# fverdoja/Fast-3D-Pointcloud-Segmentation

Hardware: AMD Instinct MI355X
Metric: Mpoints/sec segmented end-to-end, 1M-pt RGB-D frames (higher is better)
Workload: dtype f32

## Files before the change

### fast-3d-pointcloud-segmentation_amd/csrc/f3ds_algo.h

```cpp
#ifndef F3DS_ALGO_H_
#define F3DS_ALGO_H_

#include "f3ds_numerics.h"

namespace f3ds {

#define F3DS_MAX_SEED_EVENTS 48
struct SeedEvent {
    int trigger;
    int depth;
    double min[3];
    unsigned off[3];
};
struct SeedGrid {
    int n_events;
    int error;
    int defined;
    int depth;
    double res;
    double min[3], max[3];
    unsigned off[3];
    SeedEvent ev[F3DS_MAX_SEED_EVENTS];
};
F3DS_HD void a_seed_init(SeedGrid& g, float seed_res) {
// ... 126 lines not shown
    for (;;) {
        const int w = node[sp];
        const uint32_t h = s.owner[w];
        const float dw = s.dist[w];
        bool pushed = false, stolen = false;
        uint32_t g_cached = 0; bool cached_less = false;
        const bool ghosts_w = ghosts && memo[w] != (unsigned char)(T | F3DS_R_OPEN);
        for (int k = slot[sp]; k < 27; ++k) {
            int u = a_nbr_w(s, w, k);
            if (u < 0) continue;
            if (ghosts_w) {
                for (uint32_t gg = s.ghost_head[u]; gg != 0u; gg = s.ghost_next[gg])
                    if (gg < h && a_helper_dist(s, gg, w) < dw) { stolen = true; break; }
                if (stolen) break;
            }
            uint32_t g = s.owner[u];
            if (g == 0u || g >= h) continue;
            if (g != g_cached) { g_cached = g; cached_less = a_helper_dist(s, g, w) < dw; }
            if (!cached_less) continue;
            const unsigned char mu = memo[u];
            if (mu == (T | F3DS_R_TRUE)) { stolen = true; break; }
            if (mu == (T | F3DS_R_FALSE)) continue;
            slot[sp] = k + 1;
            if (sp + 1 >= F3DS_R_STACK) { *overflow = 1; return true; }
            ++sp; node[sp] = u; slot[sp] = 0;
            pushed = true;
            break;
        }
        if (pushed) continue;
        bool r = !stolen;
        for (;;) {
            memo[node[sp]] = (unsigned char)(T | (r ? F3DS_R_TRUE : F3DS_R_FALSE));
            if (sp == 0) return r;
            --sp;
            if (r) { r = false; continue; }
            break;
        }
    }
}
F3DS_HD bool a_eval_R(const SweepView& s, int w, unsigned char* memo, unsigned char tag, int* overflow, bool ghost_near = true) {
    const unsigned char T = (unsigned char)(tag << 2);
    {
        const unsigned char m0 = memo[w];
        if ((m0 & 0xFC) == T && (m0 & 3) != F3DS_R_OPEN) return (m0 & 3) == F3DS_R_TRUE;
        if (m0 == (unsigned char)(T | F3DS_R_OPEN)) ghost_near = false;
    }
    if (ghost_near && *s.n_ghosts != 0u) return a_eval_R_chain(s, w, memo, tag, overflow);
    const uint32_t h = s.owner[w];
    const float dw = s.dist[w];
    int nu[27]; uint32_t og[27];
    for (int k = 0; k < 27; ++k) nu[k] = a_nbr_w(s, w, k);
    for (int k = 0; k < 27; ++k) {
        const uint32_t g = s.owner[nu[k] >= 0 ? nu[k] : w];
        og[k] = (nu[k] >= 0 && g != 0u && g < h) ? g : 0u;
    }
    bool stolen = false, unknown = false;
    uint32_t last = 0;
    for (;;) {
        uint32_t g = 0xFFFFFFFFu;
        for (int k = 0; k < 27; ++k) if (og[k] > last && og[k] < g) g = og[k];
        if (g == 0xFFFFFFFFu) break;
        last = g;
        if (!(a_helper_dist(s, g, w) < dw)) continue;
        for (int k = 0; k < 27; ++k)
            if (og[k] == g) {
                const unsigned char mu = memo[nu[k]];
                if (mu == (T | F3DS_R_TRUE)) stolen = true;
                else if (mu != (T | F3DS_R_FALSE)) unknown = true;
            }
        if (stolen) break;
    }
    if (!stolen && unknown) return a_eval_R_chain(s, w, memo, tag, overflow);
    memo[w] = (unsigned char)(T | (stolen ? F3DS_R_FALSE : F3DS_R_TRUE));
    return !stolen;
}
#define F3DS_NO_NEXT 0x40000000u
F3DS_HD uint32_t a_umin(uint32_t a, uint32_t b) { return a < b ? a : b; }
F3DS_HD uint32_t a_umax(uint32_t a, uint32_t b) { return a > b ? a : b; }
F3DS_HD uint32_t a_next_label(const uint32_t x[27], uint32_t bias) {
    uint32_t m[9];
    for (int k = 0; k < 9; ++k) m[k] = a_umin(a_umin(x[3 * k] - bias, x[3 * k + 1] - bias), x[3 * k + 2] - bias);
    return a_umin(a_umin(a_umin(m[0], m[1]), m[2]), a_umin(a_umin(a_umin(m[3], m[4]), m[5]), a_umin(a_umin(m[6], m[7]), m[8])));
}
F3DS_HD bool a_has_thief_words(const SweepView& s, int w, uint32_t h, const uint32_t x[27]) {
    uint32_t y = a_next_label(x, 1u);
    uint32_t g = y + 1u;
    if (y >= F3DS_NO_NEXT || g >= h) return false;
    const float dw = s.dist[w];
    float wrow[12];
    a_load_row(s.vf + (size_t)w * 12, wrow);
    for (;;) {
        if (a_helper_dist_row(s, g, wrow) < dw) return true;
        const uint32_t last = g;
        y = a_next_label(x, last + 1u);
        g = y + last + 1u;
        if (y >= F3DS_NO_NEXT || g >= h) return false;
    }
}
F3DS_HD uint32_t a_thief_mask_words(const SweepView& s, int w, uint32_t h, const uint32_t x[27]) {
    uint32_t y = a_next_label(x, 1u);
    uint32_t g = y + 1u;
    if (y >= F3DS_NO_NEXT || g >= h) return 0u;
    const float dw = s.dist[w];
    float wrow[12];
    a_load_row(s.vf + (size_t)w * 12, wrow);
    uint32_t mask = 0u;
    for (;;) {
        if (a_helper_dist_row(s, g, wrow) < dw)
            for (int k = 0; k < 27; ++k) mask |= (x[k] == g ? 1u : 0u) << k;
        const uint32_t last = g;
        y = a_next_label(x, last + 1u);
        g = y + last + 1u;
        if (y >= F3DS_NO_NEXT || g >= h) return mask;
    }
}
F3DS_HD uint32_t a_thief_mask(const SweepView& s, int w) {
    const uint32_t h = s.owner[w];
    int nu[27]; uint32_t x[27];
    for (int k = 0; k < 27; ++k) nu[k] = a_nbr(s, w, k);
    for (int k = 0; k < 27; ++k) {
        const uint32_t g = s.owner[nu[k] >= 0 ? nu[k] : w];
        x[k] = nu[k] >= 0 ? g : 0u;
    }
    return a_thief_mask_words(s, w, h, x);
}
F3DS_HD bool a_ghost_steals(const SweepView& s, int w, uint32_t h) {
    const float dw = s.dist[w];
    for (int k = 0; k < 27; ++k) {
        const int u = a_nbr(s, w, k);
        if (u < 0) continue;
        for (uint32_t gg = s.ghost_head[u]; gg != 0u; gg = s.ghost_next[gg])
            if (gg < h && a_helper_dist(s, gg, w) < dw) return true;
    }
    return false;
}
#define F3DS_TMASK_GHOST 0x80000000u
F3DS_HD bool a_eval_R_mask(const SweepView& s, int w0, unsigned char* memo, unsigned char tag, const uint32_t* tmask, int* overflow) {
    const unsigned char T = (unsigned char)(tag << 2);
    {
        const unsigned char m0 = memo[w0];
        if ((m0 & 0xFC) == T && (m0 & 3) != F3DS_R_OPEN) return (m0 & 3) == F3DS_R_TRUE;
    }
    uint32_t mask0 = tmask[w0];
    if (mask0 & F3DS_TMASK_GHOST) {
        if (a_ghost_steals(s, w0, s.owner[w0])) { memo[w0] = (unsigned char)(T | F3DS_R_FALSE); return false; }
        mask0 &= ~F3DS_TMASK_GHOST;
    }
    bool stolen = false, unknown = false;
    for (uint32_t m = mask0; m != 0u; m &= m - 1u) {
        const int u = a_nbr_w(s, w0, (int)__builtin_ctz(m));
        const unsigned char mu = memo[u];
        if (mu == (unsigned char)(T | F3DS_R_TRUE)) stolen = true;
        else if (mu != (unsigned char)(T | F3DS_R_FALSE)) unknown = true;
    }
    if (stolen || !unknown) { memo[w0] = (unsigned char)(T | (stolen ? F3DS_R_FALSE : F3DS_R_TRUE)); return !stolen; }
    int node[F3DS_R_STACK];
    uint32_t rem[F3DS_R_STACK];
    int sp = 0;
    node[0] = w0; rem[0] = mask0;
    for (;;) {
        const int w = node[sp];
        bool pushed = false, st = false;
        while (rem[sp] != 0u) {
            const int k = (int)__builtin_ctz(rem[sp]);
            const int u = a_nbr_w(s, w, k);
            const unsigned char mu = memo[u];
            if (mu == (unsigned char)(T | F3DS_R_TRUE)) { st = true; break; }
            rem[sp] &= rem[sp] - 1u;
            if (mu == (unsigned char)(T | F3DS_R_FALSE)) continue;
            if (sp + 1 >= F3DS_R_STACK) { *overflow = 1; return true; }
            uint32_t mu_ = tmask[u];
            if (mu_ & F3DS_TMASK_GHOST) {
                if (a_ghost_steals(s, u, s.owner[u])) { memo[u] = (unsigned char)(T | F3DS_R_FALSE); continue; }
                mu_ &= ~F3DS_TMASK_GHOST;
            }
            ++sp; node[sp] = u; rem[sp] = mu_;
            pushed = true;
            break;
        }
        if (pushed) continue;
        bool r = !st;
        for (;;) {
            memo[node[sp]] = (unsigned char)(T | (r ? F3DS_R_TRUE : F3DS_R_FALSE));
            if (sp == 0) return r;
            --sp;
            if (r) { r = false; continue; }
            break;
        }
    }
}
F3DS_HD bool a_eval_R_step(const SweepView& s, const uint32_t* ownR, int w) {
    const uint32_t h = s.owner[w];
    if (h == 0u) return false;
    int nu[27]; uint32_t x[27];
    for (int k = 0; k < 27; ++k) nu[k] = a_nbr(s, w, k);
    for (int k = 0; k < 27; ++k) {
        const int u = nu[k] >= 0 ? nu[k] : w;
        const uint32_t g = s.owner[u], r = ownR[u];
        x[k] = (nu[k] >= 0 && (r & F3DS_OWNR_RTRUE)) ? g : 0u;
    }
    return !a_has_thief_words(s, w, h, x);
}
F3DS_HD bool a_has_thief(const SweepView& s, int w) {
    const uint32_t h = s.owner[w];
    int nu[27]; uint32_t x[27];
    for (int k = 0; k < 27; ++k) nu[k] = a_nbr(s, w, k);
    for (int k = 0; k < 27; ++k) {
        const uint32_t g = s.owner[nu[k] >= 0 ? nu[k] : w];
        x[k] = nu[k] >= 0 ? g : 0u;
    }
    return a_has_thief_words(s, w, h, x);
}
F3DS_HD void a_claim_words(const SweepView& s, int v, const uint32_t x[27], uint32_t* owner_out, float* dist_out) {
    uint32_t o = s.owner[v];
    float d = s.dist[v];
#if defined(F3DS_EXP_CLAIM_NOSEL)
    { uint32_t z = 0; for (int k = 0; k < 27; ++k) z |= x[k]; *owner_out = z == 0x7FFFFFFFu ? 1u : o; *dist_out = d; return; }
#endif
    float vrow[12];
    a_load_row(s.vf + (size_t)v * 12, vrow);
    uint32_t last = 0;
    for (;;) {
        const uint32_t y = a_next_label(x, F3DS_OWNR_RTRUE + last + 1u);
        if (y >= F3DS_NO_NEXT) break;
        const uint32_t g = y + last + 1u;
        last = g;
        if (g == o) continue;
#if defined(F3DS_EXP_CLAIM_NODIST)
        float dg = (float)g + vrow[0];
#else
        float dg = a_helper_dist_row(s, g, vrow);
#endif
        if (dg < d) { d = dg; o = g; }
    }
    *owner_out = o; *dist_out = d;
}
F3DS_HD void a_claim(const SweepView& s, const uint32_t* ownR, int v, uint32_t* owner_out, float* dist_out, unsigned char* ghost_done) {
    const bool ghosts = *s.n_ghosts != 0u;
    int nu[27]; uint32_t cand[27];
    for (int k = 0; k < 27; ++k) nu[k] = a_nbr(s, v, k);
    for (int k = 0; k < 27; ++k) {
        const uint32_t x = ownR[nu[k] >= 0 ? nu[k] : v];
        cand[k] = nu[k] >= 0 ? x : 0u;
    }
    if (!ghosts) { a_claim_words(s, v, cand, owner_out, dist_out); return; }
    for (int k = 0; k < 27; ++k) cand[k] = (cand[k] & F3DS_OWNR_RTRUE) ? (cand[k] & 0x7fffffffu) : 0u;
    uint32_t o = s.owner[v];
    float d = s.dist[v];
    float vrow[12];
    a_load_row(s.vf + (size_t)v * 12, vrow);
    uint32_t last = 0;
    for (;;) {
        uint32_t g = 0xFFFFFFFFu;
        for (int k = 0; k < 27; ++k) {
            const uint32_t gu = cand[k];
            if (gu > last && gu < g) g = gu;
        }
        for (int k = 0; k < 27; ++k) {
            const int u = a_nbr(s, v, k);
            if (u < 0) continue;
            for (uint32_t gg = s.ghost_head[u]; gg != 0u; gg = s.ghost_next[gg])
                if (gg > last && gg < g) g = gg;
        }
        if (g == 0xFFFFFFFFu) break;
        last = g;
        if (g == o) continue;
        float dg = a_helper_dist_row(s, g, vrow);
        if (dg < d) {
            d = dg; o = g;
            for (uint32_t gg = s.ghost_head[v]; gg != 0u; gg = s.ghost_next[gg])
                if (gg == g) ghost_done[g] = 1;
        }
    }
    *owner_out = o; *dist_out = d;
}
F3DS_HD void a_centroid_finish(const float sum[9], unsigned count, float row[12]) {
    float nx = sum[6], ny = sum[7], nz = sum[8];
    float z = (nx * nx + ny * ny) + (nz * nz + 0.0f);
    if (z > 0.0f) { float q = n_sqrtf(z); nx /= q; ny /= q; nz /= q; }
    float c = (float)count;
    row[0] = sum[0] / c; row[1] = sum[1] / c; row[2] = sum[2] / c;
    row[3] = sum[3] / c; row[4] = sum[4] / c; row[5] = sum[5] / c;
    row[6] = nx; row[7] = ny; row[8] = nz;
    row[9] = row[10] = row[11] = 0.0f;
}

F3DS_HD void a_payload_row(const float* vf_row, float out[12]) {
    float x = vf_row[0], y = vf_row[1], z = vf_row[2];
    out[0] = x * x; out[1] = x * y; out[2] = x * z; out[3] = y * y; out[4] = y * z; out[5] = z * z;
    out[6] = x; out[7] = y; out[8] = z;
    out[9] = (float)((uint32_t)vf_row[3] & 255u);
    out[10] = (float)((uint32_t)vf_row[4] & 255u);
    out[11] = (float)((uint32_t)vf_row[5] & 255u);
}
F3DS_HD void a_fold_row(float acc[12], const float row[12], unsigned index_plus_1) {
    for (int k = 0; k < 9; ++k) acc[k] += row[k];
    float count = (float)index_plus_1;
    float inv = 1 / count;
    for (int k = 9; k < 12; ++k) acc[k] = acc[k] + inv * (row[k] - acc[k]);
}
F3DS_HD void a_region_from_acc(const float acc[12], unsigned count, float rec[16]) {
    float c = (float)count;
    rec[0] = acc[6] / c; rec[1] = acc[7] / c; rec[2] = acc[8] / c;
    float n4[4];
    n_plane_normal(acc, count, rec, n4);
    rec[3] = n4[0]; rec[4] = n4[1]; rec[5] = n4[2];
    rec[6] = acc[9]; rec[7] = acc[10]; rec[8] = acc[11];
    n_rgb2lab(rec + 6, rec + 9);
    rec[12] = rec[13] = rec[14] = rec[15] = 0.0f;
}

struct MergeParams {
    int color_metric, geom_metric, merging;
    float lambda;
    int bins;
    const float* cdf_c;
    const float* cdf_g;
};
// ... 40 lines not shown
```

### fast-3d-pointcloud-segmentation_amd/csrc/f3ds_kernels.inc

```


namespace {

struct P16 { float x, y, z; uint32_t rgba; };

struct DevCounters {
    unsigned long long n_finite;
    uint32_t bbox[6];
    uint32_t bbox_any;
    uint32_t n_valid;
    uint32_t n_voxels;
    uint32_t n_cells;
    uint32_t n_seeds;
    uint32_t n_edges;
    uint32_t n_alive;
    uint32_t n_merges;
    uint32_t n_regions;
    uint32_t n_events;
    int error;
    int r_overflow;
    float lambda;
    uint32_t seg_count;
    uint32_t n_ghosts;
    int depth;
// ... 1787 lines not shown
    }
};
struct d_reseed_own {
    static constexpr int BLOCK = 256;
    __device__ void operator()(const int* seed, uint32_t S0, uint32_t* owner) const {
        for (uint32_t i = BIX * blockDim.x + threadIdx.x; i < S0; i += gridDim.x * blockDim.x) if (seed[i] >= 0) atomicMax(&owner[seed[i]], i + 1u);
    }
};
struct d_reseed_init {
    static constexpr int BLOCK = 256;
    __device__ void operator()(const int* seed, uint32_t S0, const uint32_t* owner, int* ghost_vox, unsigned char* ghost_active, unsigned char* ghost_done, uint32_t* hlo,
                               uint32_t* hhi, uint32_t* hcount, uint32_t* tl, uint32_t* tcnt) const {
        for (uint32_t i = BIX * blockDim.x + threadIdx.x; i <= S0; i += gridDim.x * blockDim.x) {
            ghost_done[i] = 0;
            const int v = i == 0u ? -1 : seed[i - 1];
            if (v < 0) { ghost_vox[i] = -1; ghost_active[i] = 0; hlo[i] = 0; hhi[i] = 0; hcount[i] = 0; tcnt[i] = 0; continue; }
            const bool ghost = owner[v] != i;
            ghost_vox[i] = ghost ? v : -1;
            ghost_active[i] = ghost ? 1 : 0;
            hlo[i] = (uint32_t)v; hhi[i] = (uint32_t)v; hcount[i] = 1;
            tl[(size_t)i * HT_CAP] = (uint32_t)v >> 6; tcnt[i] = ghost ? 0u : 1u;
        }
    }
};
struct SweepFrame {
    SweepView sv;
    unsigned char* R; uint32_t* ownR;
    uint32_t* owner_out; float* dist_out;
    unsigned char *ghost_done, *ghost_active; int* ghost_vox; uint32_t *ghost_head, *ghost_next;
    uint32_t *hlo, *hhi, *hcount; float* hc; DevCounters* dc; uint32_t S0;
    uint32_t *tR0, *tR1, *tC0, *tC1;
    uint32_t* tRr;
    uint32_t* hD;
    uint32_t *tl, *tcnt;
    uint32_t *wl, *wl2;
    uint32_t* tmask;
    uint32_t T, thr;
    const uint32_t *tile_n1, *tile_ord, *tile_slots;
};
template <bool ROWS = false>
__device__ inline void mark_tiles(const SweepView& s, int v, uint32_t* a, uint32_t* b, uint32_t stamp) {
#pragma unroll
    for (int k0 = 0; k0 < 27; k0 += 9) {
        int nu[9];
#pragma unroll
        for (int k = 0; k < 9; ++k) nu[k] = ROWS ? a_nbr_w(s, v, k0 + k) : a_nbr(s, v, k0 + k);
#pragma unroll
        for (int k = 0; k < 9; ++k) {
            const int u = nu[k] >= 0 ? nu[k] : v;
            a[u >> 6] = stamp; b[u >> 6] = stamp;
        }
    }
}
struct d_sweep_begin {
    static constexpr bool LATENCY_KERNEL = true;
    static constexpr int BLOCK = 256;
    __device__ void operator()(SweepFrame f, uint32_t t) const {
        __shared__ uint32_t s_n;
        if (threadIdx.x == 0) s_n = 0;
        for (uint32_t h = 1 + threadIdx.x; h <= f.S0; h += blockDim.x) if (f.ghost_vox[h] >= 0) f.ghost_head[f.ghost_vox[h]] = 0u;
        __syncthreads();
        uint32_t mine = 0;
        for (uint32_t h = 1 + threadIdx.x; h <= f.S0; h += blockDim.x)
            if (f.ghost_active[h]) { f.ghost_next[h] = atomicExch(&f.ghost_head[f.ghost_vox[h]], h); mine++; }
        if (mine) atomicAdd(&s_n, mine);
        __syncthreads();
        if (threadIdx.x == 0) {
            f.dc->n_ghosts = s_n;
            if (t == 0u) { f.dc->sweep_marks = 0u; f.dc->sweep_idle = 0u; f.dc->sweep_stats[0] = f.dc->sweep_stats[1] = f.dc->sweep_stats[2] = f.dc->sweep_stats[3] = 0u; }
            const uint32_t prev = f.dc->n_changed;
            if (t >= 2u && prev == 0u && s_n == 0u) { f.dc->sweep_idle = t + 1u; f.dc->n_changed = 0u; f.dc->sweep_stats[3]++; return; }
            if (s_n != 0u || t == 0u || prev > f.thr || f.dc->sweep_marks != t) { f.dc->sweep_full = t + 1u; f.dc->sweep_pre = t + 1u; }
            if (t != 0u && (f.thr >= 0x40000000u || prev <= 4u * f.thr)) f.dc->sweep_marks = t + 1u;
            f.dc->n_changed = 0u;
            for (int p = 0; p <= F3DS_R_PASSES; ++p) f.dc->rq[p] = 0u;
        }
    }
};
struct SweepTile {
    uint32_t (*lds)[NT_RING1 + 1];
    uint32_t (*lds2)[NT_RING1 + 1];
    int half, li;
    static constexpr int SR = (NT_RING1 + NT_TILE - 1) / NT_TILE;
    __device__ bool stage(const SweepFrame& f, uint32_t tl, const uint32_t* src, const uint32_t* src2) {
        uint32_t n1 = SW_TILE_NONE;
        if (f.tile_n1 && tl * (uint32_t)NT_TILE < (uint32_t)f.sv.V) n1 = f.tile_n1[tl];
        const bool tiled = n1 != SW_TILE_NONE;
        uint32_t a[SR], b[SR];
        if (tiled) {
            const uint32_t* ord = f.tile_ord + (size_t)tl * NT_RING1;
            uint32_t u[SR];
#pragma unroll
            for (int k = 0; k < SR; ++k) { const uint32_t i = (uint32_t)(li + k * NT_TILE); u[k] = ord[i < n1 ? i : 0u]; }
#pragma unroll
            for (int k = 0; k < SR; ++k) a[k] = src[u[k]];
            if (src2) {
#pragma unroll
                for (int k = 0; k < SR; ++k) b[k] = src2[u[k]];
            }
        }
        __syncthreads();
        if (tiled) {
#pragma unroll
            for (int k = 0; k < SR; ++k) { const uint32_t i = (uint32_t)(li + k * NT_TILE); if (i < n1) { lds[half][i] = a[k]; if (src2) lds2[half][i] = b[k]; } }
            if (li == 0) { lds[half][NT_RING1] = 0u; lds2[half][NT_RING1] = 0u; }
        }
        __syncthreads();
        return tiled;
    }
    __device__ bool stage_held(const SweepFrame& f, uint32_t tl) {
        uint32_t n1 = SW_TILE_NONE;
        if (f.tile_n1 && tl * (uint32_t)NT_TILE < (uint32_t)f.sv.V) n1 = f.tile_n1[tl];
        const bool tiled = n1 != SW_TILE_NONE;
        uint32_t g[SR], r[SR];
        if (tiled) {
            const uint32_t* ord = f.tile_ord + (size_t)tl * NT_RING1;
            uint32_t u[SR];
#pragma unroll
            for (int k = 0; k < SR; ++k) { const uint32_t i = (uint32_t)(li + k * NT_TILE); u[k] = ord[i < n1 ? i : 0u]; }
#pragma unroll
            for (int k = 0; k < SR; ++k) { g[k] = f.sv.owner[u[k]]; r[k] = f.ownR[u[k]]; }
        }
        __syncthreads();
        if (tiled) {
#pragma unroll
            for (int k = 0; k < SR; ++k) { const uint32_t i = (uint32_t)(li + k * NT_TILE); if (i < n1) lds[half][i] = (r[k] & F3DS_OWNR_RTRUE) ? g[k] : 0u; }
            if (li == 0) lds[half][NT_RING1] = 0u;
        }
        __syncthreads();
        return tiled;
    }
    __device__ void gather(const SweepFrame& f, uint32_t tl, uint32_t out[27], bool* near2) const {
        uint32_t w[SW_SLOT_WORDS];
        const uint32_t* sp = f.tile_slots + (size_t)tl * SW_SLOT_WORDS * NT_TILE + li;
#pragma unroll
        for (int k = 0; k < SW_SLOT_WORDS; ++k) w[k] = sp[k * NT_TILE];
#pragma unroll
        for (int k = 0; k < 27; ++k) out[k] = lds[half][sw_slot(w, k)];
        if (near2) {
            uint32_t any = 0u;
#pragma unroll
            for (int k = 0; k < 27; ++k) any |= lds2[half][sw_slot(w, k)];
            *near2 = any != 0u;
        }
    }
};
__device__ inline uint64_t marked_pairs(const uint32_t* stamps, uint32_t stamp, uint32_t tp0, uint32_t step, uint32_t V, uint32_t* s_marked) {
    const uint32_t k = threadIdx.x >> 2, q = threadIdx.x & 3u;
    const uint32_t v0 = (tp0 + k * step) * 256u + q * 64u;
    const bool on = v0 < V && stamps[v0 >> 6] == stamp;
    const uint64_t b = __ballot(on);
    uint32_t m16 = 0;
    for (int i = 0; i < 16; ++i) m16 |= ((uint32_t)(b >> (4 * i)) & 0xFu) ? 1u << i : 0u;
    __syncthreads();
    if (threadIdx.x < 2) s_marked[threadIdx.x] = 0u;
    __syncthreads();
    if (lane_id() == 0) atomicOr(&s_marked[threadIdx.x >> 7], m16 << (16u * ((threadIdx.x >> 6) & 1u)));
    __syncthreads();
    return (uint64_t)s_marked[0] | ((uint64_t)s_marked[1] << 32);
}
struct d_sweep_R_pre {
    static constexpr int BLOCK = 256;
    __device__ void operator()(SweepFrame f, unsigned char tag, uint32_t t) const {
        if (f.dc->sweep_full != t + 1u) return;
        __shared__ uint32_t nown[2][NT_RING1 + 1], ngh[2][NT_RING1 + 1];
        const SweepView s = f.sv;
        const bool ghosts = *s.n_ghosts != 0u;
        const int lane = lane_id();
        SweepTile st{nown, ngh, (int)(threadIdx.x >> 7), (int)(threadIdx.x & 127u)};
        for (uint32_t tp = BIX; tp * 256u < (uint32_t)s.V; tp += gridDim.x) {
            const uint32_t tl = tp * 2u + (uint32_t)st.half;
            const int v = (int)(tl * (uint32_t)NT_TILE) + st.li;
            const bool tiled = st.stage(f, tl, s.owner, ghosts ? s.ghost_head : nullptr);
            bool later = false;
            if (v < s.V) {
                const uint32_t o = s.owner[v];
                if (o == 0u) f.ownR[v] = 0u;
                else {
                    uint32_t mask;
                    if (tiled) {
                        uint32_t og[27];
                        bool near = false;
                        st.gather(f, tl, og, ghosts ? &near : nullptr);
                        mask = a_thief_mask_words(s, v, o, og) | (near ? F3DS_TMASK_GHOST : 0u);
                    } else mask = a_thief_mask(s, v) | (ghosts ? F3DS_TMASK_GHOST : 0u);
                    if (mask == 0u) { f.ownR[v] = o | F3DS_OWNR_RTRUE; f.R[v] = (unsigned char)((tag << 2) | F3DS_R_TRUE); }
                    else { f.tmask[v] = mask; later = true; }
                }
            }
            const uint64_t m = __ballot(later);
            if (m) {
                uint32_t base = 0;
                if (lane == 0) base = atomicAdd(&f.dc->rq[0], (uint32_t)__popcll(m));
                base = __builtin_amdgcn_readfirstlane(base);
                if (later) f.wl[base + (uint32_t)__popcll(m & lanemask_lt())] = (uint32_t)v;
            }
        }
    }
};
struct d_sweep_R {
    static constexpr int BLOCK = 256;
    __device__ void operator()(SweepFrame f, unsigned char tag, uint32_t t, uint32_t pass) const {
        if (f.dc->sweep_full != t + 1u) return;
        const SweepView s = f.sv;
        const uint32_t* src = (pass & 1u) ? f.wl2 : f.wl;
        uint32_t* dst = (pass & 1u) ? f.wl : f.wl2;
        if (f.dc->sweep_pre != t + 1u) {
            if (pass != 0u) return;
            for (uint32_t v = BIX * blockDim.x + threadIdx.x; v < (uint32_t)s.V; v += gridDim.x * blockDim.x) {
                const uint32_t o = s.owner[v];
                if (o == 0u) { f.ownR[v] = 0u; continue; }
                int overflow = 0;
                const bool r = a_eval_R(s, (int)v, f.R, tag, &overflow, false);
                if (!overflow) f.ownR[v] = o | (r ? F3DS_OWNR_RTRUE : 0u);
                else dst[atomicAdd(&f.dc->rq[pass + 1u], 1u)] = v;
            }
            return;
        }
        const uint32_t n = f.dc->rq[pass];
        for (uint32_t i = BIX * blockDim.x + threadIdx.x; i < n; i += gridDim.x * blockDim.x) {
            const uint32_t e = src[i];
            const int v = (int)(e & 0x7fffffffu);
            int overflow = 0;
            const uint32_t o = s.owner[v];
            const bool r = a_eval_R_mask(s, v, f.R, tag, f.tmask, &overflow);
            if (!overflow) f.ownR[v] = o | (r ? F3DS_OWNR_RTRUE : 0u);
            else dst[atomicAdd(&f.dc->rq[pass + 1u], 1u)] = e;
        }
    }
};
struct d_sweep_R_tail {
    static constexpr bool LATENCY_KERNEL = true;
    static constexpr int BLOCK = 256;
    __device__ void operator()(SweepFrame f, unsigned char tag, uint32_t t) const {
        if (f.dc->sweep_idle == t + 1u) return;
        if (threadIdx.x == 0) f.dc->sweep_stats[f.dc->sweep_full != t + 1u ? 1 : (f.dc->sweep_pre == t + 1u ? 0 : 2)]++;
        if (f.dc->sweep_full != t + 1u) return;
        __shared__ uint32_t s_n, s_next;
        const SweepView s = f.sv;
        const bool masks = f.dc->sweep_pre == t + 1u;
        uint32_t q = F3DS_R_PASSES;
        if (threadIdx.x == 0) { s_n = f.dc->rq[F3DS_R_PASSES]; s_next = 0; }
        __syncthreads();
        for (uint32_t round = 0; round < 1000000u; ++round, ++q) {
            const uint32_t n = s_n;
            if (n == 0u) break;
            const uint32_t* src = (q & 1u) ? f.wl2 : f.wl;
            uint32_t* dst = (q & 1u) ? f.wl : f.wl2;
            for (uint32_t i = threadIdx.x; i < n; i += blockDim.x) {
                const uint32_t e = src[i];
                const int v = (int)(e & 0x7fffffffu);
                int overflow = 0;
                const uint32_t o = s.owner[v];
                const bool r = masks ? a_eval_R_mask(s, v, f.R, tag, f.tmask, &overflow) : a_eval_R(s, v, f.R, tag, &overflow, false);
                if (!overflow) f.ownR[v] = o | (r ? F3DS_OWNR_RTRUE : 0u);
                else dst[atomicAdd(&s_next, 1u)] = e;
            }
            __threadfence();
            __syncthreads();
            if (threadIdx.x == 0) { if (s_next == n) f.dc->r_overflow = 1; s_n = s_next == n ? 0u : s_next; s_next = 0; }
            __syncthreads();
        }
    }
};
struct d_sweep_R_round {
    static constexpr int BLOCK = 256;
    static constexpr int WAVES_PER_SIMD = 6;
    __device__ void operator()(SweepFrame f, uint32_t t, uint32_t r, uint32_t nrounds) const {
        if (f.dc->sweep_full == t + 1u || f.dc->sweep_idle == t + 1u) return;
        __shared__ uint32_t nown[2][NT_RING1 + 1];
        const SweepView s = f.sv;
        const uint32_t stamp = t + 1u;
        const uint32_t* cur = r == 0u ? ((t & 1u) ? f.tR1 : f.tR0) : f.tRr + (size_t)(r - 1u) * f.T;
        const bool last = r + 1u == nrounds;
        uint32_t* tc = (t & 1u) ? f.tC1 : f.tC0;
        uint32_t* nxt = last ? tc : f.tRr + (size_t)r * f.T;
        SweepTile st{nown, nown, (int)(threadIdx.x >> 7), (int)(threadIdx.x & 127u)};
        __shared__ uint32_t s_marked[2];
        const uint32_t bix = BIX, step = gridDim.x;
        for (uint32_t tp0 = bix; tp0 * 256u < (uint32_t)s.V; tp0 += 64u * step)
          for (uint64_t marked = marked_pairs(cur, stamp, tp0, step, (uint32_t)s.V, s_marked); marked; marked &= marked - 1ull) {
            const uint32_t tp = tp0 + (uint32_t)__builtin_ctzll(marked) * step;
            const uint32_t tl = tp * 2u + (uint32_t)st.half;
            const int v = (int)(tl * (uint32_t)NT_TILE) + st.li;
            const bool active = v < s.V && cur[v >> 6] == stamp;
            const bool tiled = st.stage_held(f, tl);
            if (!active) continue;
            const uint32_t o = s.owner[v];
            bool keeps;
            if (tiled) {
                uint32_t og[27];
                st.gather(f, tl, og, nullptr);
                keeps = o != 0u && !a_has_thief_words(s, v, o, og);
            } else keeps = a_eval_R_step(s, f.ownR, v);
            const uint32_t nw = o | (keeps ? F3DS_OWNR_RTRUE : 0u);
            if (nw != f.ownR[v]) {
                f.ownR[v] = nw;
                mark_tiles(s, v, nxt, tc, stamp);
                if (last) f.dc->sweep_full = stamp;
            }
        }
    }
};
#ifndef F3DS_RFIRST_WPS
#define F3DS_RFIRST_WPS 6
#endif
struct d_sweep_R_first {
    static constexpr int BLOCK = 256;
    static constexpr int WAVES_PER_SIMD = F3DS_RFIRST_WPS;
    __device__ void operator()(SweepFrame f, unsigned char tag, uint32_t t, uint32_t rounds) const {
        d_sweep_R_pre{}(f, tag, t);
        if (rounds) d_sweep_R_round{}(f, t, 0u, rounds);
    }
};
struct d_sweep_claim {
    static constexpr int BLOCK = 256;
    __device__ void operator()(SweepFrame f, uint32_t t) const {
        __shared__ uint32_t nr[2][NT_RING1 + 1], ngh[2][NT_RING1 + 1];
        if (f.dc->sweep_idle == t + 1u) return;
        const SweepView s = f.sv;
        const bool full = f.dc->sweep_full == t + 1u;
        const bool marks = f.dc->sweep_marks == t + 1u;
        const bool ghosts = *s.n_ghosts != 0u;
        const uint32_t* cur = (t & 1u) ? f.tC1 : f.tC0;
        uint32_t changed = 0;
        SweepTile st{nr, ngh, (int)(threadIdx.x >> 7), (int)(threadIdx.x & 127u)};
        __shared__ uint32_t s_marked[2];
        const uint32_t bix = BIX, step = gridDim.x;
        for (uint32_t tp0 = bix; tp0 * 256u < (uint32_t)s.V; tp0 += 64u * step) {
          uint64_t marked = ~0ull;
          if (!full) marked = marked_pairs(cur, t + 1u, tp0, step, (uint32_t)s.V, s_marked);
          for (; marked; marked &= marked - 1ull) {
            const uint32_t tp = tp0 + (uint32_t)__builtin_ctzll(marked) * step;
            if (tp * 256u >= (uint32_t)s.V) break;
            const uint32_t tl = tp * 2u + (uint32_t)st.half;
            const int v = (int)(tl * (uint32_t)NT_TILE) + st.li;
            const bool active = v < s.V && (full || cur[v >> 6] == t + 1u);
            const bool tiled = st.stage(f, tl, f.ownR, ghosts ? s.ghost_head : nullptr);
            if (!active) continue;
            uint32_t o; float d;
            bool plain = false;
            if (tiled) {
                uint32_t cand[27];
                bool near = false;
                st.gather(f, tl, cand, ghosts ? &near : nullptr);
                if (!near) {
                    a_claim_words(s, v, cand, &o, &d);
                    plain = true;
                }
            }
            if (!plain) a_claim(s, f.ownR, v, &o, &d, f.ghost_done);
            const uint32_t o0 = s.owner[v];
            bool gained = false;
            if (o != o0 || __float_as_uint(d) != __float_as_uint(s.dist[v])) {
                f.owner_out[v] = o; f.dist_out[v] = d;
                if (o != o0) {
                    gained = o != 0u;
                    if (o0 != 0u) f.hD[o0] = t + 1u;
                }
                if (marks) mark_tiles(s, v, (t & 1u) ? f.tR0 : f.tR1, (t & 1u) ? f.tC0 : f.tC1, t + 2u);
                changed++;
            }
            for (uint64_t todo = __ballot(gained); todo;) {
                const int first = __builtin_ctzll(todo);
                const uint32_t og = (uint32_t)__builtin_amdgcn_readlane((int)o, first);
                const uint64_t peers = __ballot(gained && o == og);
                if (lane_id() == first) {
                    const uint32_t vmax = (uint32_t)v + (uint32_t)(63 - __builtin_clzll(peers)) - (uint32_t)first;
                    atomicMin(&f.hlo[og], (uint32_t)v); atomicMax(&f.hhi[og], vmax); f.hD[og] = t + 1u;
                    const uint32_t pos = atomicAdd(&f.tcnt[og], 1u);
                    if (pos < HT_CAP) f.tl[(size_t)og * HT_CAP + pos] = (uint32_t)v >> 6;
                }
                todo &= ~peers;
            }
          }
        }
    #pragma unroll
        for (int d = 32; d >= 1; d >>= 1) changed += __shfl_xor(changed, d, 64);
        if (lane_id() == 0 && changed) atomicAdd(&f.dc->n_changed, changed);
    }
};
__device__ inline int helper_tile_list(const uint32_t* tl, uint32_t cnt, int gv, uint32_t* srt) {
    const uint32_t n = cnt + (gv >= 0 ? 1u : 0u);
    if (cnt > HT_CAP) return -1;
    const uint32_t lane = (uint32_t)lane_id();
    if (n <= 64u) {
        uint32_t tid = 0xFFFFFFFFu;
        if (lane < cnt) tid = tl[lane];
        else if (lane == cnt && gv >= 0) tid = (uint32_t)gv >> 6;
        bool dup = lane >= n;
        for (uint32_t j = 0; j + 1u < n; ++j) { const uint32_t tj = __builtin_amdgcn_readlane(tid, j); if (j < lane && tj == tid) dup = true; }
        const uint64_t keep = __ballot(!dup);
        uint32_t rank = 0;
        for (uint64_t m = keep; m; m &= m - 1ull) { const uint32_t tj = __builtin_amdgcn_readlane(tid, (uint32_t)__builtin_ctzll(m)); rank += tj < tid; }
        if (!dup) srt[rank] = tid;
        wave_lds_sync();
        return __popcll(keep);
    }
    uint32_t nd = 0;
    for (uint32_t base = 0; base < n; base += 64u) {
        const uint32_t idx = base + lane;
        uint32_t tid = 0xFFFFFFFFu;
        if (idx < cnt) tid = tl[idx];
        else if (idx == cnt && gv >= 0) tid = (uint32_t)gv >> 6;
        bool dup = idx >= n;
        for (uint32_t j = 0; j < 64u; ++j) { const uint32_t tj = __builtin_amdgcn_readlane(tid, j); if (j < lane && tj == tid) dup = true; }
        for (uint32_t j = 0; j < nd; ++j) if (srt[j] == tid) dup = true;
        const uint64_t keep = __ballot(!dup);
        const uint32_t k = (uint32_t)__popcll(keep);
        if (nd + k > 64u) return -1;
        wave_lds_sync();
        if (!dup) srt[nd + (uint32_t)__popcll(keep & lanemask_lt())] = tid;
        nd += k;
        wave_lds_sync();
    }
    const uint32_t mine = lane < nd ? srt[lane] : 0xFFFFFFFFu;
    uint32_t rank = 0;
    for (uint32_t j = 0; j < nd; ++j) { const uint32_t tj = __builtin_amdgcn_readlane(mine, j); rank += tj < mine; }
    wave_lds_sync();
    if (lane < nd) srt[rank] = mine;
    wave_lds_sync();
    return (int)nd;
}
template <int CTRL> __device__ __forceinline__ uint32_t row_dpp_u32(uint32_t x) { return (uint32_t)__builtin_amdgcn_update_dpp((int)x, (int)x, CTRL, 0xF, 0xF, false); }
__device__ inline uint32_t row_sort16(uint32_t x, const uint32_t l16) {
#define F3DS_CX(CTRL, bit) { const uint32_t p_ = row_dpp_u32<CTRL>(x); const uint32_t lo_ = x < p_ ? x : p_, hi_ = x < p_ ? p_ : x; x = (l16 & (bit)) ? hi_ : lo_; }
    F3DS_CX(0xB1, 1u)
    F3DS_CX(0x1B, 2u) F3DS_CX(0xB1, 1u)
    F3DS_CX(0x141, 4u) F3DS_CX(0x4E, 2u) F3DS_CX(0xB1, 1u)
    F3DS_CX(0x140, 8u)
    { const uint32_t a_ = row_dpp_u32<0x12C>(x), b_ = row_dpp_u32<0x124>(x);
      const uint32_t p_ = (l16 & 4u) ? b_ : a_; const uint32_t lo_ = x < p_ ? x : p_, hi_ = x < p_ ? p_ : x; x = (l16 & 4u) ? hi_ : lo_; }
    F3DS_CX(0x4E, 2u) F3DS_CX(0xB1, 1u)
#undef F3DS_CX
    return x;
}
__device__ inline uint32_t row_leaves(const uint32_t* owner, const uint32_t V, const uint32_t h, const uint32_t tid, const int gv, uint32_t (*qt)[16], uint32_t* qleaf,
// ... 1858 lines not shown
```

Baseline: 3743.

## Prefetch tile metadata and per-point state before LDS staging barriers in sweep kernels

Splits tile staging into a request phase that loads the tile order, slot words and per-point owner, dist and feature row, and a commit phase that fills LDS. The global loads are issued before the barriers, so their latency can overlap the staging loads. Each pair's per-64-point marked stamps are cached in shared memory, so the active test no longer rereads the global stamp array. In exchange more registers are live across the barriers, which can lower occupancy.

```diff
diff --git a/fast-3d-pointcloud-segmentation_amd/csrc/f3ds_algo.h b/fast-3d-pointcloud-segmentation_amd/csrc/f3ds_algo.h
--- a/fast-3d-pointcloud-segmentation_amd/csrc/f3ds_algo.h
+++ b/fast-3d-pointcloud-segmentation_amd/csrc/f3ds_algo.h
@@ -232,11 +232,10 @@
     for (int k = 0; k < 9; ++k) m[k] = a_umin(a_umin(x[3 * k] - bias, x[3 * k + 1] - bias), x[3 * k + 2] - bias);
     return a_umin(a_umin(a_umin(m[0], m[1]), m[2]), a_umin(a_umin(a_umin(m[3], m[4]), m[5]), a_umin(a_umin(m[6], m[7]), m[8])));
 }
-F3DS_HD bool a_has_thief_words(const SweepView& s, int w, uint32_t h, const uint32_t x[27]) {
+F3DS_HD bool a_has_thief_words(const SweepView& s, int w, uint32_t h, const uint32_t x[27], float dw) {
     uint32_t y = a_next_label(x, 1u);
     uint32_t g = y + 1u;
     if (y >= F3DS_NO_NEXT || g >= h) return false;
-    const float dw = s.dist[w];
     float wrow[12];
     a_load_row(s.vf + (size_t)w * 12, wrow);
     for (;;) {
@@ -247,13 +246,18 @@
         if (y >= F3DS_NO_NEXT || g >= h) return false;
     }
 }
-F3DS_HD uint32_t a_thief_mask_words(const SweepView& s, int w, uint32_t h, const uint32_t x[27]) {
+F3DS_HD bool a_has_thief_words(const SweepView& s, int w, uint32_t h, const uint32_t x[27]) {
+    const uint32_t y = a_next_label(x, 1u);
+    if (y >= F3DS_NO_NEXT || y + 1u >= h) return false;
+    return a_has_thief_words(s, w, h, x, s.dist[w]);
+}
+F3DS_HD uint32_t a_thief_mask_words(const SweepView& s, int w, uint32_t h, const uint32_t x[27], float dw, const float* pre = nullptr) {
     uint32_t y = a_next_label(x, 1u);
     uint32_t g = y + 1u;
     if (y >= F3DS_NO_NEXT || g >= h) return 0u;
-    const float dw = s.dist[w];
     float wrow[12];
-    a_load_row(s.vf + (size_t)w * 12, wrow);
+    if (pre) { for (int k = 0; k < 12; ++k) wrow[k] = pre[k]; }
+    else a_load_row(s.vf + (size_t)w * 12, wrow);
     uint32_t mask = 0u;
     for (;;) {
         if (a_helper_dist_row(s, g, wrow) < dw)
@@ -263,6 +267,11 @@
         g = y + last + 1u;
         if (y >= F3DS_NO_NEXT || g >= h) return mask;
     }
+}
+F3DS_HD uint32_t a_thief_mask_words(const SweepView& s, int w, uint32_t h, const uint32_t x[27]) {
+    const uint32_t y = a_next_label(x, 1u);
+    if (y >= F3DS_NO_NEXT || y + 1u >= h) return 0u;
+    return a_thief_mask_words(s, w, h, x, s.dist[w]);
 }
 F3DS_HD uint32_t a_thief_mask(const SweepView& s, int w) {
     const uint32_t h = s.owner[w];
@@ -361,14 +370,10 @@
     }
     return a_has_thief_words(s, w, h, x);
 }
-F3DS_HD void a_claim_words(const SweepView& s, int v, const uint32_t x[27], uint32_t* owner_out, float* dist_out) {
-    uint32_t o = s.owner[v];
-    float d = s.dist[v];
+F3DS_HD void a_claim_words(const SweepView& s, const uint32_t x[27], uint32_t o, float d, const float vrow[12], uint32_t* owner_out, float* dist_out) {
 #if defined(F3DS_EXP_CLAIM_NOSEL)
     { uint32_t z = 0; for (int k = 0; k < 27; ++k) z |= x[k]; *owner_out = z == 0x7FFFFFFFu ? 1u : o; *dist_out = d; return; }
 #endif
-    float vrow[12];
-    a_load_row(s.vf + (size_t)v * 12, vrow);
     uint32_t last = 0;
     for (;;) {
         const uint32_t y = a_next_label(x, F3DS_OWNR_RTRUE + last + 1u);
@@ -384,6 +389,11 @@
         if (dg < d) { d = dg; o = g; }
     }
     *owner_out = o; *dist_out = d;
+}
+F3DS_HD void a_claim_words(const SweepView& s, int v, const uint32_t x[27], uint32_t* owner_out, float* dist_out) {
+    float vrow[12];
+    a_load_row(s.vf + (size_t)v * 12, vrow);
+    a_claim_words(s, x, s.owner[v], s.dist[v], vrow, owner_out, dist_out);
 }
 F3DS_HD void a_claim(const SweepView& s, const uint32_t* ownR, int v, uint32_t* owner_out, float* dist_out, unsigned char* ghost_done) {
     const bool ghosts = *s.n_ghosts != 0u;
diff --git a/fast-3d-pointcloud-segmentation_amd/csrc/f3ds_kernels.inc b/fast-3d-pointcloud-segmentation_amd/csrc/f3ds_kernels.inc
--- a/fast-3d-pointcloud-segmentation_amd/csrc/f3ds_kernels.inc
+++ b/fast-3d-pointcloud-segmentation_amd/csrc/f3ds_kernels.inc
@@ -1893,16 +1893,32 @@
     uint32_t (*lds2)[NT_RING1 + 1];
     int half, li;
     static constexpr int SR = (NT_RING1 + NT_TILE - 1) / NT_TILE;
-    __device__ bool stage(const SweepFrame& f, uint32_t tl, const uint32_t* src, const uint32_t* src2) {
-        uint32_t n1 = SW_TILE_NONE;
-        if (f.tile_n1 && tl * (uint32_t)NT_TILE < (uint32_t)f.sv.V) n1 = f.tile_n1[tl];
-        const bool tiled = n1 != SW_TILE_NONE;
+    struct Pair { uint32_t n1, ord[SR], w[SW_SLOT_WORDS]; };
+    __device__ void request(const SweepFrame& f, uint32_t tl, bool slots, Pair& q) const {
+        q.n1 = SW_TILE_NONE;
+#pragma unroll
+        for (int k = 0; k < SR; ++k) q.ord[k] = 0u;
+#pragma unroll
+        for (int k = 0; k < SW_SLOT_WORDS; ++k) q.w[k] = 0u;
+        if (f.tile_n1 && tl * (uint32_t)NT_TILE < (uint32_t)f.sv.V) {
+            q.n1 = f.tile_n1[tl];
+            const uint32_t* ord = f.tile_ord + (size_t)tl * NT_RING1;
+#pragma unroll
+            for (int k = 0; k < SR; ++k) { const uint32_t i = (uint32_t)(li + k * NT_TILE); q.ord[k] = ord[i < (uint32_t)NT_RING1 ? i : 0u]; }
+            if (slots) {
+                const uint32_t* sp = f.tile_slots + (size_t)tl * SW_SLOT_WORDS * NT_TILE + li;
+#pragma unroll
+                for (int k = 0; k < SW_SLOT_WORDS; ++k) q.w[k] = sp[k * NT_TILE];
+            }
+        }
+    }
+    __device__ bool commit(const Pair& q, const uint32_t* src, const uint32_t* src2) {
+        const bool tiled = q.n1 != SW_TILE_NONE;
         uint32_t a[SR], b[SR];
         if (tiled) {
-            const uint32_t* ord = f.tile_ord + (size_t)tl * NT_RING1;
             uint32_t u[SR];
 #pragma unroll
-            for (int k = 0; k < SR; ++k) { const uint32_t i = (uint32_t)(li + k * NT_TILE); u[k] = ord[i < n1 ? i : 0u]; }
+            for (int k = 0; k < SR; ++k) u[k] = (uint32_t)(li + k * NT_TILE) < q.n1 ? q.ord[k] : 0u;
 #pragma unroll
             for (int k = 0; k < SR; ++k) a[k] = src[u[k]];
             if (src2) {
@@ -1913,39 +1929,32 @@
         __syncthreads();
         if (tiled) {
 #pragma unroll
-            for (int k = 0; k < SR; ++k) { const uint32_t i = (uint32_t)(li + k * NT_TILE); if (i < n1) { lds[half][i] = a[k]; if (src2) lds2[half][i] = b[k]; } }
+            for (int k = 0; k < SR; ++k) { const uint32_t i = (uint32_t)(li + k * NT_TILE); if (i < q.n1) { lds[half][i] = a[k]; if (src2) lds2[half][i] = b[k]; } }
             if (li == 0) { lds[half][NT_RING1] = 0u; lds2[half][NT_RING1] = 0u; }
         }
         __syncthreads();
         return tiled;
     }
-    __device__ bool stage_held(const SweepFrame& f, uint32_t tl) {
-        uint32_t n1 = SW_TILE_NONE;
-        if (f.tile_n1 && tl * (uint32_t)NT_TILE < (uint32_t)f.sv.V) n1 = f.tile_n1[tl];
-        const bool tiled = n1 != SW_TILE_NONE;
+    __device__ bool commit_held(const SweepFrame& f, const Pair& q) {
+        const bool tiled = q.n1 != SW_TILE_NONE;
         uint32_t g[SR], r[SR];
         if (tiled) {
-            const uint32_t* ord = f.tile_ord + (size_t)tl * NT_RING1;
             uint32_t u[SR];
 #pragma unroll
-            for (int k = 0; k < SR; ++k) { const uint32_t i = (uint32_t)(li + k * NT_TILE); u[k] = ord[i < n1 ? i : 0u]; }
+            for (int k = 0; k < SR; ++k) u[k] = (uint32_t)(li + k * NT_TILE) < q.n1 ? q.ord[k] : 0u;
 #pragma unroll
             for (int k = 0; k < SR; ++k) { g[k] = f.sv.owner[u[k]]; r[k] = f.ownR[u[k]]; }
         }
         __syncthreads();
         if (tiled) {
 #pragma unroll
-            for (int k = 0; k < SR; ++k) { const uint32_t i = (uint32_t)(li + k * NT_TILE); if (i < n1) lds[half][i] = (r[k] & F3DS_OWNR_RTRUE) ? g[k] : 0u; }
+            for (int k = 0; k < SR; ++k) { const uint32_t i = (uint32_t)(li + k * NT_TILE); if (i < q.n1) lds[half][i] = (r[k] & F3DS_OWNR_RTRUE) ? g[k] : 0u; }
             if (li == 0) lds[half][NT_RING1] = 0u;
         }
         __syncthreads();
         return tiled;
     }
-    __device__ void gather(const SweepFrame& f, uint32_t tl, uint32_t out[27], bool* near2) const {
-        uint32_t w[SW_SLOT_WORDS];
-        const uint32_t* sp = f.tile_slots + (size_t)tl * SW_SLOT_WORDS * NT_TILE + li;
-#pragma unroll
-        for (int k = 0; k < SW_SLOT_WORDS; ++k) w[k] = sp[k * NT_TILE];
+    __device__ void gather(const uint32_t w[SW_SLOT_WORDS], uint32_t out[27], bool* near2) const {
 #pragma unroll
         for (int k = 0; k < 27; ++k) out[k] = lds[half][sw_slot(w, k)];
         if (near2) {
@@ -1956,6 +1965,7 @@
         }
     }
 };
+constexpr int SW_MARKED_WORDS = 2 + 8;
 __device__ inline uint64_t marked_pairs(const uint32_t* stamps, uint32_t stamp, uint32_t tp0, uint32_t step, uint32_t V, uint32_t* s_marked) {
     const uint32_t k = threadIdx.x >> 2, q = threadIdx.x & 3u;
     const uint32_t v0 = (tp0 + k * step) * 256u + q * 64u;
@@ -1965,10 +1975,15 @@
     for (int i = 0; i < 16; ++i) m16 |= ((uint32_t)(b >> (4 * i)) & 0xFu) ? 1u << i : 0u;
     __syncthreads();
     if (threadIdx.x < 2) s_marked[threadIdx.x] = 0u;
+    if (lane_id() == 0) { s_marked[2u + 2u * (threadIdx.x >> 6)] = (uint32_t)b; s_marked[3u + 2u * (threadIdx.x >> 6)] = (uint32_t)(b >> 32); }
     __syncthreads();
     if (lane_id() == 0) atomicOr(&s_marked[threadIdx.x >> 7], m16 << (16u * ((threadIdx.x >> 6) & 1u)));
     __syncthreads();
     return (uint64_t)s_marked[0] | ((uint64_t)s_marked[1] << 32);
+}
+__device__ inline bool pair_stamp(const uint32_t* s_marked, uint32_t k, uint32_t q) {
+    const uint32_t bit = 4u * k + q;
+    return (s_marked[2u + (bit >> 5)] >> (bit & 31u)) & 1u;
 }
 struct d_sweep_R_pre {
     static constexpr int BLOCK = 256;
@@ -1982,18 +1997,28 @@
         for (uint32_t tp = BIX; tp * 256u < (uint32_t)s.V; tp += gridDim.x) {
             const uint32_t tl = tp * 2u + (uint32_t)st.half;
             const int v = (int)(tl * (uint32_t)NT_TILE) + st.li;
-            const bool tiled = st.stage(f, tl, s.owner, ghosts ? s.ghost_head : nullptr);
+            SweepTile::Pair q;
+            st.request(f, tl, v < s.V, q);
+            uint32_t o = 0u; float dw = 0.0f;
+            if (v < s.V) { o = s.owner[v]; dw = s.dist[v]; }
+#if defined(F3DS_RPRE_ROW_FIRST)
+            float wrow[12] = {};
+            if (v < s.V) a_load_row(s.vf + (size_t)v * 12, wrow);
+            const float* const pre = wrow;
+#else
+            const float* const pre = nullptr;
+#endif
+            const bool tiled = st.commit(q, s.owner, ghosts ? s.ghost_head : nullptr);
             bool later = false;
             if (v < s.V) {
-                const uint32_t o = s.owner[v];
                 if (o == 0u) f.ownR[v] = 0u;
                 else {
                     uint32_t mask;
                     if (tiled) {
                         uint32_t og[27];
                         bool near = false;
-                        st.gather(f, tl, og, ghosts ? &near : nullptr);
-                        mask = a_thief_mask_words(s, v, o, og) | (near ? F3DS_TMASK_GHOST : 0u);
+                        st.gather(q.w, og, ghosts ? &near : nullptr);
+                        mask = a_thief_mask_words(s, v, o, og, dw, pre) | (near ? F3DS_TMASK_GHOST : 0u);
                     } else mask = a_thief_mask(s, v) | (ghosts ? F3DS_TMASK_GHOST : 0u);
                     if (mask == 0u) { f.ownR[v] = o | F3DS_OWNR_RTRUE; f.R[v] = (unsigned char)((tag << 2) | F3DS_R_TRUE); }
                     else { f.tmask[v] = mask; later = true; }
@@ -2087,25 +2112,29 @@
         uint32_t* tc = (t & 1u) ? f.tC1 : f.tC0;
         uint32_t* nxt = last ? tc : f.tRr + (size_t)r * f.T;
         SweepTile st{nown, nown, (int)(threadIdx.x >> 7), (int)(threadIdx.x & 127u)};
-        __shared__ uint32_t s_marked[2];
+        __shared__ uint32_t s_marked[SW_MARKED_WORDS];
         const uint32_t bix = BIX, step = gridDim.x;
         for (uint32_t tp0 = bix; tp0 * 256u < (uint32_t)s.V; tp0 += 64u * step)
           for (uint64_t marked = marked_pairs(cur, stamp, tp0, step, (uint32_t)s.V, s_marked); marked; marked &= marked - 1ull) {
-            const uint32_t tp = tp0 + (uint32_t)__builtin_ctzll(marked) * step;
+            const uint32_t pk = (uint32_t)__builtin_ctzll(marked);
+            const uint32_t tp = tp0 + pk * step;
             const uint32_t tl = tp * 2u + (uint32_t)st.half;
             const int v = (int)(tl * (uint32_t)NT_TILE) + st.li;
-            const bool active = v < s.V && cur[v >> 6] == stamp;
-            const bool tiled = st.stage_held(f, tl);
+            const bool active = v < s.V && pair_stamp(s_marked, pk, (threadIdx.x >> 6) & 3u);
+            SweepTile::Pair q;
+            st.request(f, tl, active, q);
+            uint32_t o = 0u, was = 0u; float dw = 0.0f;
+            if (active) { o = s.owner[v]; dw = s.dist[v]; was = f.ownR[v]; }
+            const bool tiled = st.commit_held(f, q);
             if (!active) continue;
-            const uint32_t o = s.owner[v];
             bool keeps;
             if (tiled) {
                 uint32_t og[27];
-                st.gather(f, tl, og, nullptr);
-                keeps = o != 0u && !a_has_thief_words(s, v, o, og);
+                st.gather(q.w, og, nullptr);
+                keeps = o != 0u && !a_has_thief_words(s, v, o, og, dw);
             } else keeps = a_eval_R_step(s, f.ownR, v);
             const uint32_t nw = o | (keeps ? F3DS_OWNR_RTRUE : 0u);
-            if (nw != f.ownR[v]) {
+            if (nw != was) {
                 f.ownR[v] = nw;
                 mark_tiles(s, v, nxt, tc, stamp);
                 if (last) f.dc->sweep_full = stamp;
@@ -2126,6 +2155,9 @@
 };
 struct d_sweep_claim {
     static constexpr int BLOCK = 256;
+#if defined(F3DS_CLAIM_WPS)
+    static constexpr int WAVES_PER_SIMD = F3DS_CLAIM_WPS;
+#endif
     __device__ void operator()(SweepFrame f, uint32_t t) const {
         __shared__ uint32_t nr[2][NT_RING1 + 1], ngh[2][NT_RING1 + 1];
         if (f.dc->sweep_idle == t + 1u) return;
@@ -2136,34 +2168,39 @@
         const uint32_t* cur = (t & 1u) ? f.tC1 : f.tC0;
         uint32_t changed = 0;
         SweepTile st{nr, ngh, (int)(threadIdx.x >> 7), (int)(threadIdx.x & 127u)};
-        __shared__ uint32_t s_marked[2];
+        __shared__ uint32_t s_marked[SW_MARKED_WORDS];
         const uint32_t bix = BIX, step = gridDim.x;
         for (uint32_t tp0 = bix; tp0 * 256u < (uint32_t)s.V; tp0 += 64u * step) {
           uint64_t marked = ~0ull;
           if (!full) marked = marked_pairs(cur, t + 1u, tp0, step, (uint32_t)s.V, s_marked);
           for (; marked; marked &= marked - 1ull) {
-            const uint32_t tp = tp0 + (uint32_t)__builtin_ctzll(marked) * step;
+            const uint32_t pk = (uint32_t)__builtin_ctzll(marked);
+            const uint32_t tp = tp0 + pk * step;
             if (tp * 256u >= (uint32_t)s.V) break;
             const uint32_t tl = tp * 2u + (uint32_t)st.half;
             const int v = (int)(tl * (uint32_t)NT_TILE) + st.li;
-            const bool active = v < s.V && (full || cur[v >> 6] == t + 1u);
-            const bool tiled = st.stage(f, tl, f.ownR, ghosts ? s.ghost_head : nullptr);
+            const bool active = v < s.V && (full || pair_stamp(s_marked, pk, (threadIdx.x >> 6) & 3u));
+            SweepTile::Pair q;
+            st.request(f, tl, active, q);
+            uint32_t o0 = 0u; float d0 = 0.0f;
+            float vrow[12] = {};
+            if (active) { o0 = s.owner[v]; d0 = s.dist[v]; a_load_row(s.vf + (size_t)v * 12, vrow); }
+            const bool tiled = st.commit(q, f.ownR, ghosts ? s.ghost_head : nullptr);
             if (!active) continue;
             uint32_t o; float d;
             bool plain = false;
             if (tiled) {
                 uint32_t cand[27];
                 bool near = false;
-                st.gather(f, tl, cand, ghosts ? &near : nullptr);
+                st.gather(q.w, cand, ghosts ? &near : nullptr);
                 if (!near) {
-                    a_claim_words(s, v, cand, &o, &d);
+                    a_claim_words(s, cand, o0, d0, vrow, &o, &d);
                     plain = true;
                 }
             }
             if (!plain) a_claim(s, f.ownR, v, &o, &d, f.ghost_done);
-            const uint32_t o0 = s.owner[v];
             bool gained = false;
-            if (o != o0 || __float_as_uint(d) != __float_as_uint(s.dist[v])) {
+            if (o != o0 || __float_as_uint(d) != __float_as_uint(d0)) {
                 f.owner_out[v] = o; f.dist_out[v] = d;
                 if (o != o0) {
                     gained = o != 0u;
```

New measurement: 3788 (median of 6 runs). No clear change (+1.2%).
